# alitteneker/jsraytracer

Measured on AMD Instinct MI355X. Metric: pixel-samples/sec + %HBM-roofline, cornell_box_path 1024² @1/2/4/8 GPU, higher is better.
Workload: dtype f64; 1 GPU; cornell_box_path 1024x1024 64spp depth 8 (Incremental); width=1024, height=1024, spp=64, max_depth=8, parallelism=tiles1, col_block=1, headline=True, gather=rgba8

## Files before the change

jsraytracer_amd/csrc/device_common.h:

```cpp
#pragma once
#include <hip/hip_runtime.h>
#include <stdint.h>

#include "device_scene.h"
#include "fdlibm.h"
#include "js_number.h"

#define JSRT_HD __host__ __device__ __forceinline__

namespace jsrt {

#define JS_PI 3.141592653589793
#define DINF __builtin_inf()

JSRT_HD bool is_nan(double x) { return x != x; }
JSRT_HD double js_max(double a, double b) {
    double r = a > b ? a : b;
    if (a == b) r = __builtin_bit_cast(double, __builtin_bit_cast(uint64_t, a) & __builtin_bit_cast(uint64_t, b));
    return a != a ? a : r;
}
JSRT_HD double js_min(double a, double b) {
    double r = a < b ? a : b;
    if (a == b) r = __builtin_bit_cast(double, __builtin_bit_cast(uint64_t, a) | __builtin_bit_cast(uint64_t, b));
    return a != a ? a : r;
// ... 35 lines not shown
    if ((x == 1.0 || x == -1.0) && __builtin_isinf(y)) return __builtin_nan("");
#ifndef JSRT_LIBM_POW
    if ((x > 0.0 || (x == 0.0 && !__builtin_signbit(x))) && x <= 2.0 && y >= 1.0 && y <= 64.0 && y == floor(y))
        return pow_int_dd(x, (int)y);
#endif
    return pow(x, y);
}
__device__ __forceinline__ double js_round(double x) {
    if (!__builtin_isfinite(x) || x == 0.0) return x;
    double r = floor(x);
    if (x - r >= 0.5) r += 1.0;
    return r;
}
JSRT_HD float or0(float x) { return (x != x || x == 0.0f) ? 0.0f : x; }

__device__ __forceinline__ uint32_t mix32(uint32_t h, uint32_t v) {
    h = (h ^ v) * 0x9E3779B1u;
    h ^= h >> 15;
    h *= 0x85EBCA77u;
    h ^= h >> 13;
    return h;
}
__device__ __forceinline__ double uniform_of(uint32_t h) {
    const uint32_t hi = mix32(h, 0xA5A5A5A5u) >> 5;
    const uint32_t lo = mix32(h, 0x5A5A5A5Au) >> 6;
    return fma((double)hi, 1.0 / 134217728.0, (double)lo * (1.0 / 9007199254740992.0));
}
__device__ __forceinline__ double keyed_uniform(uint32_t pixkey, uint32_t node, uint32_t call) {
    return uniform_of(mix32(mix32(pixkey, node), call));
}
struct Rng {
    uint32_t key, node, calls;
    __device__ __forceinline__ double next() { return keyed_uniform(key, node, calls++); }
};
struct RngH {
    uint32_t h0, calls;
    __device__ __forceinline__ double next() { return uniform_of(mix32(h0, calls++)); }
};

struct F3 {
    float x, y, z;
};
JSRT_HD F3 f3(float x, float y, float z) { return F3{x, y, z}; }
JSRT_HD F3 add(F3 a, F3 b) { return f3(a.x + b.x, a.y + b.y, a.z + b.z); }
JSRT_HD F3 sub(F3 a, F3 b) { return f3(a.x - b.x, a.y - b.y, a.z - b.z); }
JSRT_HD F3 mul(F3 a, F3 b) { return f3(a.x * b.x, a.y * b.y, a.z * b.z); }
JSRT_HD F3 scale(F3 a, double s) {
    return f3((float)((double)a.x * s), (float)((double)a.y * s), (float)((double)a.z * s));
// ... 26 lines not shown
    return f3(o.x + (float)((double)d.x * t), o.y + (float)((double)d.y * t), o.z + (float)((double)d.z * t));
}
__device__ __forceinline__ void sin_cos(double x, double &s, double &c) { fdlibm::sin_cos(x, s, c); }
constexpr double SPHERE_PICK_EPS = 0x1p-44;
JSRT_HD bool f32_stable_bits(double d) {
    const uint64_t b = __builtin_bit_cast(uint64_t, d);
    const int e = (int)((uint32_t)(b >> 52) & 0x7FFu) - 1023;
    const int sh = 8 - e;
    const uint32_t m = (uint32_t)b & 0x1FFFFFFFu;
    const uint32_t dist = m > 0x10000000u ? m - 0x10000000u : 0x10000000u - m;
    return sh <= 28 && dist > (1u << (sh < 0 ? 0 : sh));
}
struct SinCos2 {
    double st, ct, sp, cp;
};
__device__ __forceinline__ void sin_cos_of_acos(double a, double &sin_phi, double &cos_phi) {
    sin_phi = sqrt((1.0 - a) * (1.0 + a));
    cos_phi = a;
}
__device__ __forceinline__ SinCos2 sphere_pick_exact(double theta, double a) {
    SinCos2 r;
    fdlibm::sin_cos(theta, r.st, r.ct);
    fdlibm::sin_cos(fdlibm::acos(a), r.sp, r.cp);
    return r;
}
template <class R>
__device__ __forceinline__ F3 sphere_pick(R &rng) {
    const double theta = 2.0 * JS_PI * rng.next();
    const double a = 2.0 * rng.next() - 1.0;
    double sin_t, cos_t, sin_phi, cos_phi;
#ifdef JSRT_EXACT_TRIG
    const bool fast = false;
#else
    sincos(theta, &sin_t, &cos_t);
    sin_cos_of_acos(a, sin_phi, cos_phi);
    const bool fast = f32_stable_bits(cos_t * sin_phi) && f32_stable_bits(cos_phi) && f32_stable_bits(sin_t * sin_phi);
#endif
    if (__builtin_expect(!fast, 0)) {
        const SinCos2 r = sphere_pick_exact(theta, a);
        sin_t = r.st, cos_t = r.ct, sin_phi = r.sp, cos_phi = r.cp;
    }
    return f3((float)(cos_t * sin_phi), or0((float)cos_phi), or0((float)(sin_t * sin_phi)));
}
template <class R>
__device__ __forceinline__ F3 sphere_pick_fast(R &rng, bool &unstable) {
    const double theta = 2.0 * JS_PI * rng.next();
    const double a = 2.0 * rng.next() - 1.0;
    double sin_t, cos_t, sin_phi, cos_phi;
    sincos(theta, &sin_t, &cos_t);
    sin_cos_of_acos(a, sin_phi, cos_phi);
    const double px = cos_t * sin_phi, pz = sin_t * sin_phi;
    unstable = !(f32_stable_bits(px) && f32_stable_bits(cos_phi) && f32_stable_bits(pz));
    return f3((float)px, or0((float)cos_phi), or0((float)pz));
}
template <class R>
__device__ __forceinline__ F3 sphere_pick_v8(R &rng) {
    const double theta = 2.0 * JS_PI * rng.next();
    const double a = 2.0 * rng.next() - 1.0;
    double sin_t, cos_t, sin_phi, cos_phi;
    fdlibm::sin_cos(theta, sin_t, cos_t);
// ... 1388 lines not shown
            const float wx = (float)((((double)n.x * Ti[0] + (double)n.y * Ti[4]) + (double)n.z * Ti[8]) + (double)nw * Ti[12]);
            const float wy = (float)((((double)n.x * Ti[1] + (double)n.y * Ti[5]) + (double)n.z * Ti[9]) + (double)nw * Ti[13]);
            const float wz = (float)((((double)n.x * Ti[2] + (double)n.y * Ti[6]) + (double)n.z * Ti[10]) + (double)nw * Ti[14]);
            wn = normalized(f3(wx, or0(wy), or0(wz)));
        } else {
            wn = f3(Lt.wn[0], Lt.wn[1], Lt.wn[2]);
            u = local.x;
            v = local.y;
        }
        L = normalized(delta);
        const double sc = (1 / (4 * JS_PI * dot3(delta, delta))) * fabs(dot3(L, wn));
        lcol = scale(mc_eval(S, Lt.color, u, v), sc);
    }
}

__device__ __forceinline__ bool path_scatter(double mirror_prob, bool has_r, F3 R, F3 N, const ShadeData &d, Rng &rng,
                                             F3 &dir, F3 &col, uint32_t &fix, bool force) {
    fix = 0;
    if (rng.next() < mirror_prob) {
        dir = R;
        col = f3(1, 1, 1);
        return has_r;
    }
    const double dp = average3(d.diff), sp = average3(d.spec);
    const double probSum = dp + sp;
    if (probSum == 0) return false;
    if (rng.next() < (dp / probSum)) {
        const uint32_t call = rng.calls;
        bool unstable;
        const F3 sp3 = sphere_pick_fast(rng, unstable);
        if (unstable || force) fix = call + 1;
        dir = normalized(add(N, sp3));
        col = scale(d.diff, 1 / JS_PI);
        return true;
    }
    dir = R;
    col = d.spec;
    return has_r;
}


__device__ __forceinline__ void camera_ray(const DCamera &C, double x, double y, Rng &rng, F3 &o, F3 &d) {
    const double *T = C.T;
    const F3 dir = f3((float)(x * C.tan_fov * C.aspect), (float)(y * C.tan_fov), -1.0f);
    o = f3((float)T[3], (float)T[7], (float)T[11]);
    d = f3((float)((((double)dir.x * T[0] + (double)dir.y * T[1]) + (double)dir.z * T[2]) + 0.0 * T[3]),
           (float)((((double)dir.x * T[4] + (double)dir.y * T[5]) + (double)dir.z * T[6]) + 0.0 * T[7]),
           (float)((((double)dir.x * T[8] + (double)dir.y * T[9]) + (double)dir.z * T[10]) + 0.0 * T[11]));
    if (C.kind == JSRT_CAMERA_DOF) {
        const double a = rng.next() * 2 * JS_PI, rr = sqrt(rng.next());
        double sa, ca;
        sin_cos(a, sa, ca);
        const float cx = (float)(rr * ca), cy = (float)(rr * sa);
// ... 25 lines not shown
```

jsraytracer_amd/csrc/device_scene.h:

```cpp
#pragma once
#include <math.h>
#include <stdint.h>

#include <cmath>

#include "../../include/jsrt_scene.h"
#include "sdf_program.h"

namespace jsrt {

enum : int32_t { INST_PRIM = 1, INST_AGG = 2, INST_BVH = 3 };

enum : int32_t { PF_BVH = 1, PF_AGG = 2, PF_SDF = 4, PF_TRI = 8 };
enum : int32_t { PF_ANALYTIC = 0, PF_MESH = PF_BVH | PF_TRI, PF_SDF_ONLY = PF_SDF, PF_ALL = 15 };
#define PF_SDF_PROFILE PF_SDF

struct DPrim {
    double inv[12];
    int32_t gkind;
    int32_t gindex;
    int32_t material;
    int32_t casts_shadow;
    float center[4];
    float half[4];
// ... 60 lines not shown
    int32_t pos_len;
    float wn[4];
    int32_t needs_uv;
    int32_t pad2[3];
    double T[16], Ti[16];
    double inv_n;
    double pad3;
};

struct DCamera {
    double T[16];
    double tan_fov, aspect, focus, sensor;
    int32_t kind, pad[3];
};

enum { MATF_UV = 1, MATF_DIFF_CONST = 2, MATF_SPEC_CONST = 4, MATF_SPEC_ZERO = 8, MATF_PUV = 16 };

struct DScene {
    const DPrim *prims;
    const DInst *insts;
    const int32_t *inst_child;
    const int32_t *roots;
    const RootBound *rbounds;
    const DRoot *rootrec;
    const double *mats;
    const double *ctx;
    const DBvhNode *bvh;
    const int32_t *leaf_prims;
    const int32_t *leaf_tris;
    const DTri *tris;
    const DTriShade *trish;
// ... 51 lines not shown
```

jsraytracer_amd/csrc/render_kernel.h:

```cpp
#pragma once
#include <hip/hip_runtime.h>
#include <stdint.h>

#include <functional>
#include <vector>

#include "device_scene.h"

namespace jsrt {

constexpr int MAX_TREE_DEPTH = 16;
constexpr int LVL_FLAG = 63;
constexpr int LVL_UNDER = 62;
static_assert(2 * MAX_TREE_DEPTH + 2 <= LVL_UNDER, "hybrid chain count pairs lvl[2L, 2L + 1] below the flags");
constexpr int BKT_N = 64;
constexpr int BKT_S = 16;
constexpr int BKT_K = BKT_N * BKT_S;
constexpr int BKT_LEVEL = 3 * BKT_K + 64;
constexpr int HAND_PLANES = 6;

struct RenderArgs {
    int32_t W, H, kind, max_depth;
    int32_t s_begin, s_end, spp;
    uint32_t seed;
// ... 31 lines not shown
    uint8_t *endl;
    uint32_t *qctr;
    uint4 *fixrec;
    uint32_t *fixctr;
    uint32_t fixcap;
    int32_t force_fix;
    float4 *sray;
    float4 *scol;
    uint32_t *bkt;
    uint32_t *bbase;
    uint32_t *brank;
    uint32_t p0, npix, s0, npaths;
    int32_t ns;
    int32_t group;
    int32_t shadow_node;
    int32_t chain;
    int32_t hybrid;
    uint32_t cap;
    int32_t bucket;
    int32_t child_sort;
    int32_t bucket_grid;
    int32_t pixel_major;
    size_t pool, level_cap;
    size_t nstride, hstride;
    size_t sstride;
};

struct RayFeed {
    const float *rays;
    const uint32_t *keys;
// ... 97 lines not shown
```

jsraytracer_amd/csrc/render_levels.h:

```cpp
#pragma once
#include <hip/hip_runtime.h>
#include <stdint.h>
#include <stdlib.h>
#include <string.h>

#include <algorithm>
#include <type_traits>
#include <vector>

#include "device_common.h"
#include "render_kernel.h"
#include "render_plan.h"

#ifndef JSRT_SHADE_OCC
#define JSRT_SHADE_OCC 4
#endif
#ifndef JSRT_SHADE_OCC_SDF
#define JSRT_SHADE_OCC_SDF 3
#endif
#ifndef JSRT_SHADE_OCC_FLAT
#define JSRT_SHADE_OCC_FLAT 5
#endif
#ifndef JSRT_SHADOW_OCC
#define JSRT_SHADOW_OCC 6
// ... 133 lines not shown

__device__ __forceinline__ void write_result(const WArgs &W, uint32_t i, F3 c) {
    const uint32_t p = W.parent[i];
    if (p == DEAD_RAY) return;
    if (p == NO_PARENT) {
        float *dst = W.root + 3 * (size_t)W.path[i];
        dst[0] = c.x;
        dst[1] = c.y;
        dst[2] = c.z;
    } else {
        W.slot[(size_t)(p & 1u) * W.nstride + (p >> 1)] = make_float4(c.x, c.y, c.z, 0.0f);
    }
}


__device__ __forceinline__ F3 pick(bool f, F3 a, F3 b) { return f3(f ? a.x : b.x, f ? a.y : b.y, f ? a.z : b.z); }
__device__ __forceinline__ Child pick(bool f, const Child &a, const Child &b) {
    return Child{pick(f, a.dir, b.dir), pick(f, a.col, b.col), pick(f, a.w, b.w), f ? a.k : b.k};
}

struct LevelRange {
    uint32_t base, count;
};
__device__ __forceinline__ LevelRange level_range(const WArgs &W, int L) {
    if (W.lvl[LVL_FLAG]) return LevelRange{0u, 0u};
    uint32_t b = 0;
    for (int j = 0; j < L; ++j) b += W.lvl[j];
    return LevelRange{b, W.lvl[L]};
}
__device__ __forceinline__ LevelRange chain_level(const WArgs &W, int L) {
    const uint32_t base = (uint32_t)L * W.cap;
    if (!W.hybrid) return LevelRange{base, W.npaths};
    if (W.lvl[LVL_FLAG]) return LevelRange{base, 0u};
    return LevelRange{base, W.lvl[2 * L] + W.lvl[2 * L + 1]};
// ... 2 lines not shown
    uint32_t c = W.npaths;
    for (int j = 1; j < L; ++j) c += as_const(W.lvl)[2 * j + 1];
    return c;
}
__device__ __forceinline__ uint32_t chain_slot(const WArgs &W, int L, uint32_t t) {
    if (!W.hybrid || L == 0) return t;
    const uint32_t nc = as_const(W.lvl)[2 * L];
    return t < nc ? ((L & 1) ? W.list1 : W.list0)[t] : side_base(W, L) + (t - nc);
}

constexpr uint32_t HAND_KR = 0x80000000u;
constexpr uint32_t HAND_DIFF = 0x40000000u;
constexpr uint32_t HAND_R = 0x20000000u;
constexpr uint32_t HAND_SPEC = 0x10000000u;
constexpr uint32_t HAND_MAT = 0x0FFFFF00u;

struct Handoff {
    F3 pos, N, R, refr, diff, spec;
    double kr;
    int32_t mkind, mat;
    uint32_t addr, key;
    uint32_t node;
    uint32_t mask;
    uint32_t flags;
};
struct NodeOut {
    F3 surf;
    uint32_t info;

    Handoff h;
// ... 155 lines not shown
        const float wx = (float)((((double)nrm.x * inv[0] + (double)nrm.y * inv[4]) + (double)nrm.z * inv[8]) + (double)nrm_w * inv[12]);
        const float wy = (float)((((double)nrm.x * inv[1] + (double)nrm.y * inv[5]) + (double)nrm.z * inv[9]) + (double)nrm_w * inv[13]);
        const float wz = (float)((((double)nrm.x * inv[2] + (double)nrm.y * inv[6]) + (double)nrm.z * inv[10]) + (double)nrm_w * inv[14]);
        sf.N = normalized(f3(wx, or0(wy), or0(wz)));
    }
    sf.u = u;
    sf.v = v;
    sf.basecolor = basecolor;
    sf.bary = bary;
    sf.has_uv = has_uv;
    sf.has_bc = has_bc;
    sf.has_bary = has_bary;
}

constexpr uint32_t INFO_FIX = 1u << 30;
template <int PF, bool TEX, bool PUV = false>
__device__ __forceinline__ int shade_node(const DScene &S, bool lit, const Hit &h, F3 o, F3 d, uint32_t addr,
                                          uint32_t key, NodeOut &out, Child &ch0, Child &ch1, uint32_t *fixl,
                                          bool force_fix) {
    const DPrim &P = S.prims[h.prim];
    Surface sf;
    const bool puv = PUV && (S.mat_flags[P.material] & MATF_PUV) != 0;
    surface_data<PF, false>(S, h, o, d, (S.mat_flags[P.material] & MATF_UV) != 0 && !puv, sf);
    const F3 N = sf.N, basecolor = sf.basecolor;
    float u = sf.u, v = sf.v;
    ShadeData sd;
    sd.pos = ray_point(o, d, h.t);
    if constexpr (PUV) {
        if (puv && (S.mat_flags[P.material] & MATF_UV)) posuv_map(S.puv[P.material], sd.pos.x, sd.pos.y, sd.pos.z, u, v);
    }
    out.h.pos = sd.pos;
// ... 60 lines not shown
    uint32_t info = INFO_HIT;
    if (lit) {
        info |= INFO_LIT;
        out.h.N = sd.N;
        out.h.R = sd.R;
        out.h.refr = sd.refr;
        out.h.diff = sd.diff;
        out.h.spec = sd.spec;
        out.h.kr = sd.kr;
        out.h.mkind = mkind;
        out.h.mat = P.material;
        const int32_t mf = S.mat_flags[P.material];
        uint32_t fl = 0;
        if (!(mf & MATF_DIFF_CONST) || sf.has_bc) fl |= HAND_DIFF;
        if (!(mf & MATF_SPEC_CONST)) fl |= HAND_SPEC;
        if (mkind != JSRT_MAT_PHONG && sd.kr != 1.0) fl |= HAND_KR | HAND_R;
        if (!(mf & MATF_SPEC_ZERO) || !(__builtin_isfinite(sd.R.x) && __builtin_isfinite(sd.R.y) && __builtin_isfinite(sd.R.z)))
            fl |= HAND_R;
        out.h.flags = fl;
        rng.calls = (uint32_t)S.light_draws;
    }
    int n = 0;
    uint32_t fix0 = 0u, fix1 = 0u;
    auto push = [&](const Child &c) {
        const bool first = n == 0;
        ch0 = pick(first, c, ch0);
        ch1 = pick(first, ch1, c);
        ++n;
    };
    if (mkind == JSRT_MAT_PHONG) {
        if (dot3(sd.refl, sd.refl) > 0) push(Child{sd.R, f3(1, 1, 1), sd.refl, 1.0});
        if (dot3(sd.trans, sd.trans) > 0) push(Child{normalized(d), f3(1, 1, 1), sd.trans, 1.0});
    } else {
        if (sd.kr > 0) {
            F3 dir = sd.R, col = f3(1, 1, 1);
            bool ok = true;
            uint32_t fx = 0;
            if (mkind == JSRT_MAT_PATH) ok = path_scatter(M.mirror_prob, true, sd.R, Nn, sd, rng, dir, col, fx, force_fix);
            if (ok) {
                fix0 = fx;
                push(Child{dir, col, sd.refl, sd.kr});
            }
        }
        if (sd.kr < 1) {
            F3 dir = sd.refr, col = f3(1, 1, 1);
            bool ok = sd.has_refr;
            uint32_t fx = 0;
            if (mkind == JSRT_MAT_PATH) ok = path_scatter(M.mirror_prob, sd.has_refr, sd.refr, neg(Nn), sd, rng, dir, col, fx, force_fix);
            if (ok) {
                if (fx) {
                    if (n == 0) fix0 = fx | 0x80000000u;
                    else fix1 = fx | 0x80000000u;
                }
                push(Child{dir, col, sd.trans, 1 - sd.kr});
            }
        }
    }
    if (__builtin_expect((fix0 | fix1) != 0u, 0)) {
        const uint32_t t = threadIdx.x;
        fixl[t] = fix0;
        fixl[256 + t] = fix1;
        fixl[512 + t] = __float_as_uint(Nn.x);
        fixl[768 + t] = __float_as_uint(Nn.y);
        fixl[1024 + t] = __float_as_uint(Nn.z);
        info |= INFO_FIX;
    }
    out.info = info | ((uint32_t)n << INFO_NCHILD_SHIFT);
    return n;
}

__device__ __forceinline__ float u2f(uint32_t x) { return __uint_as_float(x); }
__device__ __forceinline__ uint32_t f2u(float x) { return __float_as_uint(x); }

// ... 6 lines not shown
__device__ __forceinline__ void store_child(const WArgs &W, uint32_t i, uint32_t j, const Child &c) {
    float4 *x = W.child + (size_t)(2 * j) * W.nstride + i;
    x[0] = make_float4(c.col.x, c.col.y, c.col.z, c.w.x);
    if (!unit_child(c))
        x[W.nstride] = make_float4(c.w.y, c.w.z, u2f((uint32_t)__double2loint(c.k)), u2f((uint32_t)__double2hiint(c.k)));
}
__device__ __forceinline__ F3 add_child(const WArgs &W, uint32_t i, uint32_t j, F3 c, F3 v, uint32_t info,
                                       const float4 *first = nullptr) {
    const float4 *x = W.child + (size_t)(2 * j) * W.nstride + i;
    const float4 a = first ? *first : x[0];
    if (info & (j == 0 ? INFO_UNIT0 : INFO_UNIT1)) return add(c, mul(v, f3(a.x, a.y, a.z)));
    const float4 b = x[W.nstride];
    const double k = __hiloint2double((int)f2u(b.w), (int)f2u(b.z));
    return add(c, scale(mul(mul(v, f3(a.x, a.y, a.z)), f3(a.w, b.x, b.y)), k));
}
__device__ __forceinline__ void store_hand(const WArgs &W, uint32_t h, const Handoff &o) {
    float4 *p = W.hand + h;
    const size_t hs = W.hstride;
    const uint32_t fl = o.flags;
    const uint32_t tag = ((uint32_t)o.mat << 8) | (o.mask & 0xFFu) | fl;
    p[0] = make_float4(o.pos.x, o.pos.y, o.pos.z, u2f(mix32(o.key, o.addr)));
    p[hs] = make_float4(o.N.x, o.N.y, o.N.z, u2f(tag));
    if (fl & HAND_DIFF) p[2 * hs] = make_float4(o.diff.x, o.diff.y, o.diff.z, 0.0f);
    if (fl & HAND_R) p[3 * hs] = make_float4(o.R.x, o.R.y, o.R.z, u2f((uint32_t)__double2hiint(o.kr)));
    if (fl & HAND_SPEC) p[4 * hs] = make_float4(o.spec.x, o.spec.y, o.spec.z, 0.0f);
    if (fl & HAND_KR) p[5 * hs] = make_float4(o.refr.x, o.refr.y, o.refr.z, u2f((uint32_t)__double2loint(o.kr)));
    if (W.bucket) W.hnode[h] = o.node;
}

__device__ __forceinline__ F3 accumulate(const RenderArgs &A, F3 acc, F3 col) {
    if (A.kind == JSRT_RENDERER_RANDOM) return add(acc, scale(col, 1.0 / A.spp));
    if (A.kind == JSRT_RENDERER_INCREMENTAL) return f3(acc.x + col.x, acc.y + or0(col.y), acc.z + or0(col.z));
    return col;
}

// ... 120 lines not shown
    SL.prims = reinterpret_cast<const DPrim *>(sb + SL.stab_off[STAB_PRIMS]);
    SL.prim_shade = reinterpret_cast<const int32_t *>(sb + SL.stab_off[STAB_PRIM_SHADE]);
    SL.shade0 = reinterpret_cast<const double *>(sb + SL.stab_off[STAB_SHADE0]);
    SL.shadeI = reinterpret_cast<const double *>(sb + SL.stab_off[STAB_SHADEI]);
    SL.prim_lit = reinterpret_cast<const int32_t *>(sb + SL.stab_off[STAB_PRIM_LIT]);
    SL.puv = reinterpret_cast<const jsrt_rec_posuv *>(sb + SL.stab_off[STAB_POSUV]);
}
__device__ __forceinline__ void stab_stage(const DScene &S, DScene &SL, int words, bool shade) {
    extern __shared__ uint4 stab_lds[];
    const uint4 *src = reinterpret_cast<const uint4 *>(S.stab);
    for (int k = (int)threadIdx.x; k < words; k += 256) stab_lds[k] = src[k];
    __syncthreads();
    stab_bind(SL, stab_lds, shade);
}

template <int PF, bool CHAIN, bool STAGE, bool TEX = false, bool PUV = false>
__global__ __launch_bounds__(256, PF == PF_ANALYTIC ? JSRT_SHADE_OCC_FLAT
                                                    : (PF & PF_SDF) ? JSRT_SHADE_OCC_SDF : JSRT_SHADE_OCC) SHADE_ATTR void k_shade(
    DScene S, WArgs W, int L, int child_depth) {
    const uint32_t t0 = blockIdx.x * 256, tt = t0 + threadIdx.x;
    const LevelRange R = CHAIN ? chain_level(W, L) : level_range(W, L);
    const uint32_t count = R.count, base = R.base, next_base = CHAIN ? 0u : R.base + R.count;
    if (!CHAIN || W.hybrid || STAGE) {
        if (t0 >= count) return;
    } else if (tt >= count) {
        return;
    }
    const bool in = tt < count;
    const uint32_t q = in ? tt : 0u;
    const uint32_t slot = CHAIN && in ? chain_slot(W, L, q) : q;
    const uint32_t i = base + (CHAIN ? slot : q);
    const uint32_t r = CHAIN ? slot : i;
    int nchild = 0;
    Child ch0, ch1;
// ... 18 lines not shown
    uint32_t parent = 0, path = 0, hslot = ~0u;
    if (!CHAIN && prim != NO_RAY) {
        parent = W.parent[r];
        path = W.path[r];
    }
    if (hit) {
        if (!STAGE) {
            ro = f3(W.ox[r], W.oy[r], W.oz[r]);
            rd = f3(W.dx[r], W.dy[r], W.dz[r]);
            rt = W.t[r];
            rctx = W.ctx[r];
            raddr = W.addr[r];
            rkey = W.key[r];
        }
        const Hit h{rt, prim, rctx};
        nchild = shade_node<PF, TEX, PUV>(SL, W.ns > 0, h, ro, rd, raddr, rkey, out, ch0, ch1, fixl, W.force_fix != 0);
        out.h.node = CHAIN ? slot : q;
        out.h.mask = (uint32_t)S.grid_cells;
        if (W.bucket && (out.info & INFO_LIT)) {
            const uint32_t br = W.brank[r];
            const int b = (int)(br >> 16);
            const uint32_t *B = W.bkt + (size_t)L * BKT_LEVEL;
            hslot = B[2 * BKT_K + bucket_key(W, b)] + W.bbase[(size_t)blockIdx.x * BKT_N + b] + (br & 0xFFFFu);
            if (hslot >= B[3 * BKT_K]) hslot = ~0u;
            if (W.bucket_grid) out.h.mask = (uint32_t)b;
        }
    }
    uint32_t co[2] = {0u, 1u};
    uint32_t at = 0, side_at = 0;
    if (!CHAIN) {
        const int nc = child_depth > 0 ? nchild : 0;
        if (W.child_sort)
            at = block_append_keyed(W.lvl + L + 1, nc, nchild > 0 ? octant(ch0.dir) : 0, nchild > 1 ? octant(ch1.dir) : 0,
                                    co[0], co[1]);
        else
            at = block_append<256>(W.lvl + L + 1, nc);
    } else if (W.hybrid) {
        const int side = (child_depth > 0 && nchild > 1) ? 1 : 0, cont = (child_depth > 0 && nchild > 0) ? 1 : 0;
        block_append2(W.lvl + 2 * (L + 1), cont, side, at, side_at);
        side_at += side_base(W, L + 1);
    }
    if (__builtin_expect(hit && (out.info & INFO_FIX) != 0u, 0) && child_depth > 0) {
        if (CHAIN) fix_record(W, fixl, out.h.key, out.h.addr, W.hybrid ? nchild : 1, r, side_at);
        else fix_record(W, fixl, out.h.key, out.h.addr, nchild, next_base + at + co[0], next_base + at + co[1]);
    }
    if (prim == NO_RAY) {
        if (in) store_node(W, i, f3(0, 0, 0), 0u);
        if (CHAIN && W.hybrid && in) W.endl[r] = (uint8_t)L;
        return;
    }
    if (!hit) {
        const F3 bg = f3(S.bg[0], S.bg[1], S.bg[2]);
        if (CHAIN) {
            store_node(W, i, bg, INFO_MISS);
            W.prim[r] = NO_RAY;
            if (W.hybrid) W.endl[r] = (uint8_t)L;
        } else {
            if (parent == NO_PARENT) {
                float *dst = W.root + 3 * (size_t)path;
                dst[0] = bg.x;
                dst[1] = bg.y;
                dst[2] = bg.z;
            } else if (parent != DEAD_RAY) {
                W.slot[(size_t)(parent & 1u) * W.nstride + (parent >> 1)] = make_float4(bg.x, bg.y, bg.z, 0.0f);
            }
            store_node(W, i, bg, 0u);
        }
        return;
    }
    if (nchild > 0 && unit_child(ch0)) out.info |= INFO_UNIT0;
    if (nchild > 1 && unit_child(ch1)) out.info |= INFO_UNIT1;
    store_node(W, i, out.surf, out.info & ~INFO_FIX);
    if (out.info & INFO_LIT) {
        if (!W.bucket) store_hand(W, q, out.h);
        else if (hslot != ~0u) store_hand(W, hslot, out.h);
    }
    if (nchild > 0) store_child(W, i, 0, ch0);
    if (nchild > 1) store_child(W, i, 1, ch1);
    if (CHAIN) {
        uint32_t *next = (L & 1) ? W.list0 : W.list1;
        if (child_depth > 0 && nchild > 0) {
            W.ox[r] = out.h.pos.x; W.oy[r] = out.h.pos.y; W.oz[r] = out.h.pos.z;
            W.dx[r] = ch0.dir.x; W.dy[r] = ch0.dir.y; W.dz[r] = ch0.dir.z;
            W.addr[r] = mix32(out.h.addr, 1u);
            if (W.hybrid) next[at] = r;
        } else {
            W.prim[r] = NO_RAY;
            if (W.hybrid) W.endl[r] = (uint8_t)L;
        }
        if (W.hybrid && child_depth > 0 && nchild > 1) {
// ... 29 lines not shown
        W.dx[rr] = c.dir.x; W.dy[rr] = c.dir.y; W.dz[rr] = c.dir.z;
        W.addr[rr] = mix32(out.h.addr, (uint32_t)j + 1);
        W.key[rr] = out.h.key;
        W.path[rr] = path;
        W.parent[rr] = 2 * i + (uint32_t)j;
        W.prim[rr] = -1;
    }
}


__device__ __forceinline__ F3 mc_const3(const DScene &S, int m) {
    const float4 c = *reinterpret_cast<const float4 *>(S.mc_const + 4 * m);
    return f3(c.x, c.y, c.z);
}
__device__ __forceinline__ bool hand_decode(const DScene &S, const float4 &h1, const float4 *hp, size_t hs, ShadeData &sd,
                                            int &mkind) {
    const uint32_t tag = f2u(h1.w);
    const jsrt_rec_material &M = S.mat[(tag & HAND_MAT) >> 8];
    sd.N = f3(h1.x, h1.y, h1.z);
    sd.diff = (tag & HAND_DIFF) ? f3(hp[2 * hs].x, hp[2 * hs].y, hp[2 * hs].z) : mc_const3(S, M.diffuse);
    sd.spec = (tag & HAND_SPEC) ? f3(hp[4 * hs].x, hp[4 * hs].y, hp[4 * hs].z) : mc_const3(S, M.specular);
    sd.R = f3(0, 0, 0);
    sd.refr = f3(0, 0, 0);
    sd.kr = 1.0;
    if (tag & HAND_R) {
        const float4 h3 = hp[3 * hs];
        sd.R = f3(h3.x, h3.y, h3.z);
        if (tag & HAND_KR) {
            const float4 h5 = hp[5 * hs];
            sd.refr = f3(h5.x, h5.y, h5.z);
            sd.kr = __hiloint2double((int)f2u(h3.w), (int)f2u(h5.w));
        }
    }
// ... 124 lines not shown
    const LevelRange R = CHAIN ? chain_level(W, L) : level_range(W, L);
    const uint32_t count = R.count, base = R.base;
    const uint32_t ns = (uint32_t)W.ns;
    const uint32_t e = blockIdx.x * 256 + threadIdx.x;
    const bool in = e < as_const(W.bkt + (size_t)L * BKT_LEVEL)[3 * BKT_K];
    const uint32_t h = in ? e : 0u;
    const float4 *hp = W.hand + h;
    const size_t hs = W.hstride;
    const uint32_t q = W.hnode[h];
    const float4 h0 = hp[0], h1 = hp[hs];
    const uint32_t tag = f2u(h1.w);
    uint64_t mask = ~0ull;
    if (W.bucket_grid && S.grid_masked) mask = wave_root_mask(S, tag & 0xFFu, in);
    const bool lit = in && q < (CHAIN ? W.cap : count);
    const uint32_t i = base + (lit ? q : 0u);
    const float4 nd = W.node[i];
    DScene SL = S;
    stab_stage(S, SL, S.stab_words_shadow, false);
    if (!lit) return;
    const F3 P = f3(h0.x, h0.y, h0.z);
    ShadeData sd;
    int mkind;
    const bool no_r = hand_decode(SL, h1, hp, hs, sd, mkind);
    F3 d[NS], c[NS];
    uint32_t live = 0u;
#pragma unroll
    for (int s = 0; s < NS; ++s) {
        d[s] = f3(1, 1, 1);
        c[s] = f3(0, 0, 0);
        if ((uint32_t)s < ns) {
            RngH rng{f2u(h0.w), (uint32_t)SL.sample_call[s]};
            F3 Ld, lcol;
            light_sample<false>(SL, as_const(S.lights)[0], P, rng, d[s], Ld, lcol);
            c[s] = light_sample_color(mkind, sd, Ld, lcol, no_r);
            if (!(c[s].x == 0.0f && c[s].y == 0.0f && c[s].z == 0.0f)) live |= 1u << s;
        }
    }
    live = world_any_node<PF, NS>(S, P, d, live, 0.0001, 1, mask);
// ... 270 lines not shown
            v = sf.v;
            hu = 1;
        }
    }
    uv[2 * (size_t)i] = u;
    uv[2 * (size_t)i + 1] = v;
    has[i] = hu;
}
template <int PF>
void material_uv_pf(const DScene &S, const float *rays, uint32_t n, float *uv, int32_t *has, hipStream_t st) {
    const size_t lds = (PF & (PF_BVH | PF_AGG)) ? bvh_lds_bytes(S, 256) : 0;
    hipLaunchKernelGGL((k_material_uv<PF>), dim3(grid_ub(n)), dim3(256), lds, st, S, rays, n, uv, has);
}

template <int PF, bool CHAIN>
void run_batch(const DScene &S, const RenderArgs &A, const WArgs &W, hipStream_t st, KernelTimes *kt,
               const std::vector<size_t> &bound, const BatchSync *sync) {
    auto accum_wait = [&] { if (sync && sync->wait) (void)hipStreamWaitEvent(st, sync->wait, 0); };
    auto accum_done = [&] { if (sync && sync->done) (void)hipEventRecord(sync->done, st); };
    const hipStream_t ss = (sync && sync->aux) ? sync->aux : st;
    const bool split = ss != st;
    auto timed = [&](int which, auto launch) {
        const bool ev = kt && kt->on(which);
        const hipStream_t s = which == KT_SHADOW ? ss : st;
        if (ev) kt->ev[which].begin(s);
        launch();
        if (ev) kt->ev[which].end(s);
    };
    const size_t lds = (PF & (PF_BVH | PF_AGG)) ? bvh_lds_bytes(S, 256) : 0;
    const bool Q = (PF & PF_SDF) && W.sstride != 0;
    if (Q) (void)hipMemsetAsync(W.qctr, 0, 64 * sizeof(uint32_t), st);
    if (W.bucket) (void)hipMemsetAsync(W.bkt, 0, (size_t)MAX_TREE_DEPTH * BKT_LEVEL * sizeof(uint32_t), st);
// ... 13 lines not shown
        timed(KT_EXTEND, [&] {
            if (Q && S.sdf_all_forms)
                hipLaunchKernelGGL((k_extend_q<PF, CHAIN, true>), dim3(persistent_grid((const void *)k_extend_q<PF, CHAIN, true>, ub)),
                                   dim3(256), 0, st, S, W, L, L == 0 ? 0.0 : 0.0001);
            else if (Q)
                hipLaunchKernelGGL((k_extend_q<PF, CHAIN, false>), dim3(persistent_grid((const void *)k_extend_q<PF, CHAIN, false>, ub)),
                                   dim3(256), 0, st, S, W, L, L == 0 ? 0.0 : 0.0001);
            else
                hipLaunchKernelGGL((k_extend<PF, CHAIN>), dim3(grid_ub(ub)), dim3(256), lds, st, S, W, L, L == 0 ? 0.0 : 0.0001);
        });
        if (W.bucket) hipLaunchKernelGGL(k_bucket_offsets, dim3(1), dim3(256), 0, st, W, L);
        if (split && L > 0 && W.ns > 0) (void)hipStreamWaitEvent(st, sync->shadow_done, 0);
        timed(KT_SHADE, [&] {
            const bool staged = PF == PF_ANALYTIC && S.stab_words > 0;
            const size_t sl = staged ? (size_t)S.stab_words * 16 : 0;
            if (S.has_posuv) {
                if (staged)
                    hipLaunchKernelGGL((k_shade<PF, CHAIN, PF == PF_ANALYTIC, true, true>), dim3(grid_ub(ub)), dim3(256), sl, st, S, W, L, child_depth);
                else
                    hipLaunchKernelGGL((k_shade<PF, CHAIN, false, true, true>), dim3(grid_ub(ub)), dim3(256), 0, st, S, W, L, child_depth);
            } else if (S.has_textures) {
                if (staged)
                    hipLaunchKernelGGL((k_shade<PF, CHAIN, PF == PF_ANALYTIC, true>), dim3(grid_ub(ub)), dim3(256), sl, st, S, W, L, child_depth);
                else
                    hipLaunchKernelGGL((k_shade<PF, CHAIN, false, true>), dim3(grid_ub(ub)), dim3(256), 0, st, S, W, L, child_depth);
            } else if (staged)
                hipLaunchKernelGGL((k_shade<PF, CHAIN, PF == PF_ANALYTIC>), dim3(grid_ub(ub)), dim3(256), sl, st, S, W, L, child_depth);
            else
                hipLaunchKernelGGL((k_shade<PF, CHAIN, false>), dim3(grid_ub(ub)), dim3(256), 0, st, S, W, L, child_depth);
            if (child_depth > 0) hipLaunchKernelGGL(k_fix_dirs, dim3(1), dim3(256), 0, st, W);
// ... 19 lines not shown
                const size_t sl = (size_t)S.stab_words_shadow * 16;
                auto shadow = [&](auto serial, auto stage) {
                    constexpr bool SERIAL = decltype(serial)::value, STAGE = decltype(stage)::value;
                    const dim3 g(grid_ub(SERIAL ? ub : ne));
                    const size_t l = STAGE ? sl : lds;
                    if (S.sphere_lights)
                        hipLaunchKernelGGL((k_shadow<PF, CHAIN, SERIAL, true, STAGE>), g, dim3(256), l, ss, S, W, L);
                    else
                        hipLaunchKernelGGL((k_shadow<PF, CHAIN, SERIAL, false, STAGE>), g, dim3(256), l, ss, S, W, L);
                };
                constexpr bool FLAT_PF = PF == PF_ANALYTIC;
                if (W.ns > 1 && W.group <= 1) {
                    shadow(std::true_type{}, std::false_type{});
                } else if (FLAT_PF && sl) {
                    if constexpr (FLAT_PF) {
                        if (W.shadow_node && W.bucket && S.n_lights == 1 && !S.sphere_lights && W.ns > 1 && W.ns <= 4) {
                            hipLaunchKernelGGL((k_shadow_node<PF, CHAIN, 4>), dim3(grid_ub(ub)), dim3(256), sl, ss, S, W, L);
                            return;
                        }
                    }
                    shadow(std::false_type{}, std::bool_constant<FLAT_PF>{});
                } else {
                    shadow(std::false_type{}, std::false_type{});
                }
            });
        if (W.ns > 0 && split) (void)hipEventRecord(sync->shadow_done, ss);
    }
    if (split && W.ns > 0 && !ubs.empty()) (void)hipStreamWaitEvent(st, sync->shadow_done, 0);
    if (CHAIN && W.hybrid) {
        timed(KT_RESOLVE, [&] {
            if (ubs.empty()) {
// ... 36 lines not shown
```

jsraytracer_amd/csrc/scene_load.cpp:

```cpp
#include "scene_load.h"

#include <float.h>
#include <math.h>
#include <string.h>

#include <algorithm>
#include <map>
#include <set>
#include <unordered_map>

namespace jsrt {
namespace {

struct Blob {
    const jsrt_rec_renderer *rndr = nullptr;
    const jsrt_rec_camera *cam = nullptr;
    const jsrt_rec_mcolor *mc = nullptr;
    const jsrt_rec_material *mat = nullptr;
    const jsrt_rec_geometry *geom = nullptr;
    const jsrt_rec_object *obj = nullptr;
    const jsrt_rec_matrix *mats = nullptr;
    const int32_t *root = nullptr, *chld = nullptr;
    const jsrt_rec_bvhnode *bvh = nullptr;
    const jsrt_rec_triangle *tri = nullptr;
// ... 1029 lines not shown
                check_mc((int32_t)i);
                S.has_textures = 1;
            }
        }
        if (S.has_textures) {
            S.tex.assign(B.tex, B.tex + B.n_tex);
            S.texels.assign(B.texl, B.texl + B.n_texl);
            for (int b = 0; b < 256; ++b) S.tex_q255.push_back((double)b / 255.0);
        }
        mc_constants();
        for (size_t i = 0; i < S.mat.size(); ++i) {
            const jsrt_rec_material &M = S.mat[i];
            if (M.kind == JSRT_MAT_SOLID || M.kind == JSRT_MAT_TRANSPARENT) continue;
            const float *d = &S.mc_const[4 * (size_t)M.diffuse], *sp = &S.mc_const[4 * (size_t)M.specular];
            if (d[3] != 0.0f) S.mat_flags[i] |= MATF_DIFF_CONST;
            if (sp[3] != 0.0f) {
                S.mat_flags[i] |= MATF_SPEC_CONST;
                uint32_t b[3];
                memcpy(b, sp, sizeof b);
                if (b[0] == 0u && b[1] == 0u && b[2] == 0u && M.smoothness >= 0.0 && M.smoothness <= 1e5)
                    S.mat_flags[i] |= MATF_SPEC_ZERO;
            }
        }

        const double I[16] = {1, 0, 0, 0, 0, 1, 0, 0, 0, 0, 1, 0, 0, 0, 0, 1};
        for (int k = 0; k < 16; ++k) S.ctx.push_back(I[k]);
        S.all_roots_prims = 1;
        for (uint32_t i = 0; i < B.n_root; ++i) {
            const int32_t ix = inst(B.root[i], I, 0);
            S.roots.push_back(ix);
// ... 248 lines not shown
```

Before: 676.7 million pixel-samples/s.

## Skip node store via handoff tag packing and specialize last-level shade kernel

For the analytic flat pipeline with a single light and bucketed shadow-node path, the shade kernel now packs the child count and unit bits, plus an ambient-needed flag, into the handoff tag. The shadow-node kernel rebuilds the node word from that tag and from the constant material ambient, so the separate node store and load is skipped when ambient is constant. A LAST template specialization of k_shade for child_depth==0 skips child appends, fix records and direction sampling while still advancing the RNG call counter. The price is more template instantiations and a tighter material-index field in the tag.

```diff
diff --git a/jsraytracer_amd/csrc/device_common.h b/jsraytracer_amd/csrc/device_common.h
--- a/jsraytracer_amd/csrc/device_common.h
+++ b/jsraytracer_amd/csrc/device_common.h
@@ -73,24 +73,24 @@
 }
 JSRT_HD float or0(float x) { return (x != x || x == 0.0f) ? 0.0f : x; }
 
-__device__ __forceinline__ uint32_t mix32(uint32_t h, uint32_t v) {
+JSRT_HD uint32_t mix32(uint32_t h, uint32_t v) {
     h = (h ^ v) * 0x9E3779B1u;
     h ^= h >> 15;
     h *= 0x85EBCA77u;
     h ^= h >> 13;
     return h;
 }
-__device__ __forceinline__ double uniform_of(uint32_t h) {
+JSRT_HD double uniform_of(uint32_t h) {
     const uint32_t hi = mix32(h, 0xA5A5A5A5u) >> 5;
     const uint32_t lo = mix32(h, 0x5A5A5A5Au) >> 6;
     return fma((double)hi, 1.0 / 134217728.0, (double)lo * (1.0 / 9007199254740992.0));
 }
-__device__ __forceinline__ double keyed_uniform(uint32_t pixkey, uint32_t node, uint32_t call) {
+JSRT_HD double keyed_uniform(uint32_t pixkey, uint32_t node, uint32_t call) {
     return uniform_of(mix32(mix32(pixkey, node), call));
 }
 struct Rng {
     uint32_t key, node, calls;
-    __device__ __forceinline__ double next() { return keyed_uniform(key, node, calls++); }
+    JSRT_HD double next() { return keyed_uniform(key, node, calls++); }
 };
 struct RngH {
     uint32_t h0, calls;
@@ -147,7 +147,7 @@
 struct SinCos2 {
     double st, ct, sp, cp;
 };
-__device__ __forceinline__ void sin_cos_of_acos(double a, double &sin_phi, double &cos_phi) {
+JSRT_HD void sin_cos_of_acos(double a, double &sin_phi, double &cos_phi) {
     sin_phi = sqrt((1.0 - a) * (1.0 + a));
     cos_phi = a;
 }
@@ -176,7 +176,7 @@
     return f3((float)(cos_t * sin_phi), or0((float)cos_phi), or0((float)(sin_t * sin_phi)));
 }
 template <class R>
-__device__ __forceinline__ F3 sphere_pick_fast(R &rng, bool &unstable) {
+JSRT_HD F3 sphere_pick_fast(R &rng, bool &unstable) {
     const double theta = 2.0 * JS_PI * rng.next();
     const double a = 2.0 * rng.next() - 1.0;
     double sin_t, cos_t, sin_phi, cos_phi;
@@ -1595,8 +1595,9 @@
     }
 }
 
-__device__ __forceinline__ bool path_scatter(double mirror_prob, bool has_r, F3 R, F3 N, const ShadeData &d, Rng &rng,
-                                             F3 &dir, F3 &col, uint32_t &fix, bool force) {
+template <bool NODIR = false>
+JSRT_HD bool path_scatter(double mirror_prob, bool has_r, F3 R, F3 N, const ShadeData &d, Rng &rng, F3 &dir, F3 &col,
+                          uint32_t &fix, bool force) {
     fix = 0;
     if (rng.next() < mirror_prob) {
         dir = R;
@@ -1607,17 +1608,71 @@
     const double probSum = dp + sp;
     if (probSum == 0) return false;
     if (rng.next() < (dp / probSum)) {
-        const uint32_t call = rng.calls;
-        bool unstable;
-        const F3 sp3 = sphere_pick_fast(rng, unstable);
-        if (unstable || force) fix = call + 1;
-        dir = normalized(add(N, sp3));
+        if constexpr (NODIR) {
+            rng.calls += 2;
+            dir = N;
+        } else {
+            const uint32_t call = rng.calls;
+            bool unstable;
+            const F3 sp3 = sphere_pick_fast(rng, unstable);
+            if (unstable || force) fix = call + 1;
+            dir = normalized(add(N, sp3));
+        }
         col = scale(d.diff, 1 / JS_PI);
         return true;
     }
     dir = R;
     col = d.spec;
     return has_r;
+}
+
+JSRT_HD F3 pick(bool f, F3 a, F3 b) { return f3(f ? a.x : b.x, f ? a.y : b.y, f ? a.z : b.z); }
+JSRT_HD Child pick(bool f, const Child &a, const Child &b) {
+    return Child{pick(f, a.dir, b.dir), pick(f, a.col, b.col), pick(f, a.w, b.w), f ? a.k : b.k};
+}
+template <bool NODIR = false>
+JSRT_HD int scatter_children(int mkind, double mirror_prob, const ShadeData &sd, F3 d, Rng &rng, bool force_fix,
+                             Child &ch0, Child &ch1, uint32_t &fix0, uint32_t &fix1) {
+    const F3 Nn = sd.N;
+    int n = 0;
+    fix0 = 0u;
+    fix1 = 0u;
+    auto push = [&](const Child &c) {
+        const bool first = n == 0;
+        ch0 = pick(first, c, ch0);
+        ch1 = pick(first, ch1, c);
+        ++n;
+    };
+    if (mkind == JSRT_MAT_PHONG) {
+        if (dot3(sd.refl, sd.refl) > 0) push(Child{sd.R, f3(1, 1, 1), sd.refl, 1.0});
+        if (dot3(sd.trans, sd.trans) > 0) push(Child{NODIR ? sd.R : normalized(d), f3(1, 1, 1), sd.trans, 1.0});
+    } else {
+        if (sd.kr > 0) {
+            F3 dir = sd.R, col = f3(1, 1, 1);
+            bool ok = true;
+            uint32_t fx = 0;
+            if (mkind == JSRT_MAT_PATH) ok = path_scatter<NODIR>(mirror_prob, true, sd.R, Nn, sd, rng, dir, col, fx, force_fix);
+            if (ok) {
+                fix0 = fx;
+                push(Child{dir, col, sd.refl, sd.kr});
+            }
+        }
+        if (sd.kr < 1) {
+            F3 dir = sd.refr, col = f3(1, 1, 1);
+            bool ok = sd.has_refr;
+            uint32_t fx = 0;
+            if (mkind == JSRT_MAT_PATH)
+                ok = path_scatter<NODIR>(mirror_prob, sd.has_refr, sd.refr, neg(Nn), sd, rng, dir, col, fx, force_fix);
+            if (ok) {
+                if (fx) {
+                    if (n == 0) fix0 = fx | 0x80000000u;
+                    else fix1 = fx | 0x80000000u;
+                }
+                push(Child{dir, col, sd.trans, 1 - sd.kr});
+            }
+        }
+    }
+    return n;
 }
 
 
diff --git a/jsraytracer_amd/csrc/device_scene.h b/jsraytracer_amd/csrc/device_scene.h
--- a/jsraytracer_amd/csrc/device_scene.h
+++ b/jsraytracer_amd/csrc/device_scene.h
@@ -98,7 +98,7 @@
     int32_t kind, pad[3];
 };
 
-enum { MATF_UV = 1, MATF_DIFF_CONST = 2, MATF_SPEC_CONST = 4, MATF_SPEC_ZERO = 8, MATF_PUV = 16 };
+enum { MATF_UV = 1, MATF_DIFF_CONST = 2, MATF_SPEC_CONST = 4, MATF_SPEC_ZERO = 8, MATF_PUV = 16, MATF_AMB_CONST = 32 };
 
 struct DScene {
     const DPrim *prims;
diff --git a/jsraytracer_amd/csrc/render_kernel.h b/jsraytracer_amd/csrc/render_kernel.h
--- a/jsraytracer_amd/csrc/render_kernel.h
+++ b/jsraytracer_amd/csrc/render_kernel.h
@@ -69,6 +69,7 @@
     int32_t ns;
     int32_t group;
     int32_t shadow_node;
+    int32_t node_single;
     int32_t chain;
     int32_t hybrid;
     uint32_t cap;
diff --git a/jsraytracer_amd/csrc/render_levels.h b/jsraytracer_amd/csrc/render_levels.h
--- a/jsraytracer_amd/csrc/render_levels.h
+++ b/jsraytracer_amd/csrc/render_levels.h
@@ -171,10 +171,6 @@
 }
 
 
-__device__ __forceinline__ F3 pick(bool f, F3 a, F3 b) { return f3(f ? a.x : b.x, f ? a.y : b.y, f ? a.z : b.z); }
-__device__ __forceinline__ Child pick(bool f, const Child &a, const Child &b) {
-    return Child{pick(f, a.dir, b.dir), pick(f, a.col, b.col), pick(f, a.w, b.w), f ? a.k : b.k};
-}
 
 struct LevelRange {
     uint32_t base, count;
@@ -207,6 +203,18 @@
 constexpr uint32_t HAND_R = 0x20000000u;
 constexpr uint32_t HAND_SPEC = 0x10000000u;
 constexpr uint32_t HAND_MAT = 0x0FFFFF00u;
+constexpr uint32_t HAND_MAT1 = 0x007FFF00u;
+constexpr uint32_t HAND_AMB = 0x00800000u;
+constexpr int HAND_INFO_SHIFT = 24;
+static_assert((size_t)STAB_MAX_WORDS * 16 / sizeof(int32_t) <= (HAND_MAT1 >> 8) + 1, "a staged scene's materials fit HAND_MAT1");
+static_assert(INFO_NCHILD_SHIFT == 2 && INFO_UNIT0 == 32u && INFO_UNIT1 == 64u, "hand_info's packing");
+__device__ __forceinline__ uint32_t hand_info(uint32_t info) {
+    return (((info >> INFO_NCHILD_SHIFT) & 3u) | ((info >> 3) & 0xCu)) << HAND_INFO_SHIFT;
+}
+__device__ __forceinline__ uint32_t hand_info_word(uint32_t tag) {
+    const uint32_t p = tag >> HAND_INFO_SHIFT;
+    return INFO_HIT | INFO_LIT | ((p & 3u) << INFO_NCHILD_SHIFT) | ((p & 0xCu) << 3);
+}
 
 struct Handoff {
     F3 pos, N, R, refr, diff, spec;
@@ -392,7 +400,7 @@
 }
 
 constexpr uint32_t INFO_FIX = 1u << 30;
-template <int PF, bool TEX, bool PUV = false>
+template <int PF, bool TEX, bool PUV = false, bool NODIR = false>
 __device__ __forceinline__ int shade_node(const DScene &S, bool lit, const Hit &h, F3 o, F3 d, uint32_t addr,
                                           uint32_t key, NodeOut &out, Child &ch0, Child &ch1, uint32_t *fixl,
                                           bool force_fix) {
@@ -483,49 +491,55 @@
         uint32_t fl = 0;
         if (!(mf & MATF_DIFF_CONST) || sf.has_bc) fl |= HAND_DIFF;
         if (!(mf & MATF_SPEC_CONST)) fl |= HAND_SPEC;
+        if constexpr (PF == PF_ANALYTIC)
+            if (!(mf & MATF_AMB_CONST) || sf.has_bc) fl |= HAND_AMB;
         if (mkind != JSRT_MAT_PHONG && sd.kr != 1.0) fl |= HAND_KR | HAND_R;
         if (!(mf & MATF_SPEC_ZERO) || !(__builtin_isfinite(sd.R.x) && __builtin_isfinite(sd.R.y) && __builtin_isfinite(sd.R.z)))
             fl |= HAND_R;
         out.h.flags = fl;
         rng.calls = (uint32_t)S.light_draws;
     }
+    uint32_t fix0 = 0u, fix1 = 0u;
     int n = 0;
-    uint32_t fix0 = 0u, fix1 = 0u;
-    auto push = [&](const Child &c) {
-        const bool first = n == 0;
-        ch0 = pick(first, c, ch0);
-        ch1 = pick(first, ch1, c);
-        ++n;
-    };
-    if (mkind == JSRT_MAT_PHONG) {
-        if (dot3(sd.refl, sd.refl) > 0) push(Child{sd.R, f3(1, 1, 1), sd.refl, 1.0});
-        if (dot3(sd.trans, sd.trans) > 0) push(Child{normalized(d), f3(1, 1, 1), sd.trans, 1.0});
+    if constexpr (PF == PF_ANALYTIC) {
+        n = scatter_children<NODIR>(mkind, M.mirror_prob, sd, d, rng, force_fix, ch0, ch1, fix0, fix1);
     } else {
-        if (sd.kr > 0) {
-            F3 dir = sd.R, col = f3(1, 1, 1);
-            bool ok = true;
-            uint32_t fx = 0;
-            if (mkind == JSRT_MAT_PATH) ok = path_scatter(M.mirror_prob, true, sd.R, Nn, sd, rng, dir, col, fx, force_fix);
-            if (ok) {
-                fix0 = fx;
-                push(Child{dir, col, sd.refl, sd.kr});
+        auto push = [&](const Child &c) {
+            const bool first = n == 0;
+            ch0 = pick(first, c, ch0);
+            ch1 = pick(first, ch1, c);
+            ++n;
+        };
+        if (mkind == JSRT_MAT_PHONG) {
+            if (dot3(sd.refl, sd.refl) > 0) push(Child{sd.R, f3(1, 1, 1), sd.refl, 1.0});
+            if (dot3(sd.trans, sd.trans) > 0) push(Child{normalized(d), f3(1, 1, 1), sd.trans, 1.0});
+        } else {
+            if (sd.kr > 0) {
+                F3 dir = sd.R, col = f3(1, 1, 1);
+                bool ok = true;
+                uint32_t fx = 0;
+                if (mkind == JSRT_MAT_PATH) ok = path_scatter(M.mirror_prob, true, sd.R, Nn, sd, rng, dir, col, fx, force_fix);
+                if (ok) {
+                    fix0 = fx;
+                    push(Child{dir, col, sd.refl, sd.kr});
+                }
             }
-        }
-        if (sd.kr < 1) {
-            F3 dir = sd.refr, col = f3(1, 1, 1);
-            bool ok = sd.has_refr;
-            uint32_t fx = 0;
-            if (mkind == JSRT_MAT_PATH) ok = path_scatter(M.mirror_prob, sd.has_refr, sd.refr, neg(Nn), sd, rng, dir, col, fx, force_fix);
-            if (ok) {
-                if (fx) {
-                    if (n == 0) fix0 = fx | 0x80000000u;
-                    else fix1 = fx | 0x80000000u;
+            if (sd.kr < 1) {
+                F3 dir = sd.refr, col = f3(1, 1, 1);
+                bool ok = sd.has_refr;
+                uint32_t fx = 0;
+                if (mkind == JSRT_MAT_PATH) ok = path_scatter(M.mirror_prob, sd.has_refr, sd.refr, neg(Nn), sd, rng, dir, col, fx, force_fix);
+                if (ok) {
+                    if (fx) {
+                        if (n == 0) fix0 = fx | 0x80000000u;
+                        else fix1 = fx | 0x80000000u;
+                    }
+                    push(Child{dir, col, sd.trans, 1 - sd.kr});
                 }
-                push(Child{dir, col, sd.trans, 1 - sd.kr});
             }
         }
     }
-    if (__builtin_expect((fix0 | fix1) != 0u, 0)) {
+    if (!NODIR && __builtin_expect((fix0 | fix1) != 0u, 0)) {
         const uint32_t t = threadIdx.x;
         fixl[t] = fix0;
         fixl[256 + t] = fix1;
@@ -562,11 +576,13 @@
     const double k = __hiloint2double((int)f2u(b.w), (int)f2u(b.z));
     return add(c, scale(mul(mul(v, f3(a.x, a.y, a.z)), f3(a.w, b.x, b.y)), k));
 }
-__device__ __forceinline__ void store_hand(const WArgs &W, uint32_t h, const Handoff &o) {
+template <bool FLAT>
+__device__ __forceinline__ void store_hand(const WArgs &W, uint32_t h, const Handoff &o, uint32_t info) {
     float4 *p = W.hand + h;
     const size_t hs = W.hstride;
-    const uint32_t fl = o.flags;
-    const uint32_t tag = ((uint32_t)o.mat << 8) | (o.mask & 0xFFu) | fl;
+    const uint32_t fl = FLAT ? o.flags & ~HAND_AMB : o.flags;
+    uint32_t tag = ((uint32_t)o.mat << 8) | (o.mask & 0xFFu) | fl;
+    if (FLAT && W.node_single) tag |= (o.flags & HAND_AMB) | hand_info(info);
     p[0] = make_float4(o.pos.x, o.pos.y, o.pos.z, u2f(mix32(o.key, o.addr)));
     p[hs] = make_float4(o.N.x, o.N.y, o.N.z, u2f(tag));
     if (fl & HAND_DIFF) p[2 * hs] = make_float4(o.diff.x, o.diff.y, o.diff.z, 0.0f);
@@ -717,10 +733,11 @@
     stab_bind(SL, stab_lds, shade);
 }
 
-template <int PF, bool CHAIN, bool STAGE, bool TEX = false, bool PUV = false>
+template <int PF, bool CHAIN, bool STAGE, bool TEX = false, bool PUV = false, bool LAST = false>
 __global__ __launch_bounds__(256, PF == PF_ANALYTIC ? JSRT_SHADE_OCC_FLAT
                                                     : (PF & PF_SDF) ? JSRT_SHADE_OCC_SDF : JSRT_SHADE_OCC) SHADE_ATTR void k_shade(
-    DScene S, WArgs W, int L, int child_depth) {
+    DScene S, WArgs W, int L, int child_depth_arg) {
+    const int child_depth = LAST ? 0 : child_depth_arg;
     const uint32_t t0 = blockIdx.x * 256, tt = t0 + threadIdx.x;
     const LevelRange R = CHAIN ? chain_level(W, L) : level_range(W, L);
     const uint32_t count = R.count, base = R.base, next_base = CHAIN ? 0u : R.base + R.count;
@@ -769,7 +786,7 @@
             rkey = W.key[r];
         }
         const Hit h{rt, prim, rctx};
-        nchild = shade_node<PF, TEX, PUV>(SL, W.ns > 0, h, ro, rd, raddr, rkey, out, ch0, ch1, fixl, W.force_fix != 0);
+        nchild = shade_node<PF, TEX, PUV, LAST>(SL, W.ns > 0, h, ro, rd, raddr, rkey, out, ch0, ch1, fixl, W.force_fix != 0);
         out.h.node = CHAIN ? slot : q;
         out.h.mask = (uint32_t)S.grid_cells;
         if (W.bucket && (out.info & INFO_LIT)) {
@@ -783,7 +800,8 @@
     }
     uint32_t co[2] = {0u, 1u};
     uint32_t at = 0, side_at = 0;
-    if (!CHAIN) {
+    if (LAST) {
+    } else if (!CHAIN) {
         const int nc = child_depth > 0 ? nchild : 0;
         if (W.child_sort)
             at = block_append_keyed(W.lvl + L + 1, nc, nchild > 0 ? octant(ch0.dir) : 0, nchild > 1 ? octant(ch1.dir) : 0,
@@ -795,7 +813,7 @@
         block_append2(W.lvl + 2 * (L + 1), cont, side, at, side_at);
         side_at += side_base(W, L + 1);
     }
-    if (__builtin_expect(hit && (out.info & INFO_FIX) != 0u, 0) && child_depth > 0) {
+    if (!LAST && __builtin_expect(hit && (out.info & INFO_FIX) != 0u, 0) && child_depth > 0) {
         if (CHAIN) fix_record(W, fixl, out.h.key, out.h.addr, W.hybrid ? nchild : 1, r, side_at);
         else fix_record(W, fixl, out.h.key, out.h.addr, nchild, next_base + at + co[0], next_base + at + co[1]);
     }
@@ -825,10 +843,12 @@
     }
     if (nchild > 0 && unit_child(ch0)) out.info |= INFO_UNIT0;
     if (nchild > 1 && unit_child(ch1)) out.info |= INFO_UNIT1;
-    store_node(W, i, out.surf, out.info & ~INFO_FIX);
-    if (out.info & INFO_LIT) {
-        if (!W.bucket) store_hand(W, q, out.h);
-        else if (hslot != ~0u) store_hand(W, hslot, out.h);
+    const uint32_t info = out.info & ~INFO_FIX;
+    const bool by_shadow = PF == PF_ANALYTIC && W.node_single && (info & INFO_LIT) && !(out.h.flags & HAND_AMB) && hslot != ~0u;
+    if (!by_shadow) store_node(W, i, out.surf, info);
+    if (info & INFO_LIT) {
+        if (!W.bucket) store_hand<PF == PF_ANALYTIC>(W, q, out.h, info);
+        else if (hslot != ~0u) store_hand<PF == PF_ANALYTIC>(W, hslot, out.h, info);
     }
     if (nchild > 0) store_child(W, i, 0, ch0);
     if (nchild > 1) store_child(W, i, 1, ch1);
@@ -888,9 +908,9 @@
     return f3(c.x, c.y, c.z);
 }
 __device__ __forceinline__ bool hand_decode(const DScene &S, const float4 &h1, const float4 *hp, size_t hs, ShadeData &sd,
-                                            int &mkind) {
+                                            int &mkind, uint32_t matmask = HAND_MAT) {
     const uint32_t tag = f2u(h1.w);
-    const jsrt_rec_material &M = S.mat[(tag & HAND_MAT) >> 8];
+    const jsrt_rec_material &M = S.mat[(tag & matmask) >> 8];
     sd.N = f3(h1.x, h1.y, h1.z);
     sd.diff = (tag & HAND_DIFF) ? f3(hp[2 * hs].x, hp[2 * hs].y, hp[2 * hs].z) : mc_const3(S, M.diffuse);
     sd.spec = (tag & HAND_SPEC) ? f3(hp[4 * hs].x, hp[4 * hs].y, hp[4 * hs].z) : mc_const3(S, M.specular);
@@ -1045,14 +1065,23 @@
     if (W.bucket_grid && S.grid_masked) mask = wave_root_mask(S, tag & 0xFFu, in);
     const bool lit = in && q < (CHAIN ? W.cap : count);
     const uint32_t i = base + (lit ? q : 0u);
-    const float4 nd = W.node[i];
+    const bool single = W.node_single != 0;
+    float4 nd = make_float4(0.0f, 0.0f, 0.0f, 0.0f);
+    if (!single || (lit && (tag & HAND_AMB))) nd = W.node[i];
     DScene SL = S;
     stab_stage(S, SL, S.stab_words_shadow, false);
     if (!lit) return;
     const F3 P = f3(h0.x, h0.y, h0.z);
     ShadeData sd;
     int mkind;
-    const bool no_r = hand_decode(SL, h1, hp, hs, sd, mkind);
+    const bool no_r = hand_decode(SL, h1, hp, hs, sd, mkind, single ? HAND_MAT1 : HAND_MAT);
+    if (single) {
+        if (!(tag & HAND_AMB)) {
+            const F3 amb = mc_const3(SL, SL.mat[(tag & HAND_MAT1) >> 8].ambient);
+            nd.x = amb.x, nd.y = amb.y, nd.z = amb.z;
+        }
+        nd.w = u2f(hand_info_word(tag));
+    }
     F3 d[NS], c[NS];
     uint32_t live = 0u;
 #pragma unroll
@@ -1353,8 +1382,12 @@
 }
 
 template <int PF, bool CHAIN>
-void run_batch(const DScene &S, const RenderArgs &A, const WArgs &W, hipStream_t st, KernelTimes *kt,
+void run_batch(const DScene &S, const RenderArgs &A, const WArgs &pool_args, hipStream_t st, KernelTimes *kt,
                const std::vector<size_t> &bound, const BatchSync *sync) {
+    const bool node_form = PF == PF_ANALYTIC && S.stab_words_shadow > 0 && pool_args.shadow_node && pool_args.bucket &&
+                           S.n_lights == 1 && !S.sphere_lights && pool_args.ns > 1 && pool_args.ns <= 4 && pool_args.group > 1;
+    WArgs W = pool_args;
+    W.node_single = node_form ? 1 : 0;
     auto accum_wait = [&] { if (sync && sync->wait) (void)hipStreamWaitEvent(st, sync->wait, 0); };
     auto accum_done = [&] { if (sync && sync->done) (void)hipEventRecord(sync->done, st); };
     const hipStream_t ss = (sync && sync->aux) ? sync->aux : st;
@@ -1398,6 +1431,20 @@
         timed(KT_SHADE, [&] {
             const bool staged = PF == PF_ANALYTIC && S.stab_words > 0;
             const size_t sl = staged ? (size_t)S.stab_words * 16 : 0;
+            if constexpr (PF == PF_ANALYTIC) {
+                if (child_depth == 0) {
+                    auto last = [&](auto stage, auto tex, auto puv) {
+                        constexpr bool ST = decltype(stage)::value, TX = decltype(tex)::value, PU = decltype(puv)::value;
+                        hipLaunchKernelGGL((k_shade<PF, CHAIN, ST, TX, PU, true>), dim3(grid_ub(ub)), dim3(256), ST ? sl : 0, st, S, W, L, 0);
+                    };
+                    using T = std::true_type;
+                    using F = std::false_type;
+                    if (S.has_posuv) staged ? last(T{}, T{}, T{}) : last(F{}, T{}, T{});
+                    else if (S.has_textures) staged ? last(T{}, T{}, F{}) : last(F{}, T{}, F{});
+                    else staged ? last(T{}, F{}, F{}) : last(F{}, F{}, F{});
+                    return;
+                }
+            }
             if (S.has_posuv) {
                 if (staged)
                     hipLaunchKernelGGL((k_shade<PF, CHAIN, PF == PF_ANALYTIC, true, true>), dim3(grid_ub(ub)), dim3(256), sl, st, S, W, L, child_depth);
@@ -1447,7 +1494,7 @@
                     shadow(std::true_type{}, std::false_type{});
                 } else if (FLAT_PF && sl) {
                     if constexpr (FLAT_PF) {
-                        if (W.shadow_node && W.bucket && S.n_lights == 1 && !S.sphere_lights && W.ns > 1 && W.ns <= 4) {
+                        if (node_form) {
                             hipLaunchKernelGGL((k_shadow_node<PF, CHAIN, 4>), dim3(grid_ub(ub)), dim3(256), sl, ss, S, W, L);
                             return;
                         }
diff --git a/jsraytracer_amd/csrc/scene_load.cpp b/jsraytracer_amd/csrc/scene_load.cpp
--- a/jsraytracer_amd/csrc/scene_load.cpp
+++ b/jsraytracer_amd/csrc/scene_load.cpp
@@ -1067,6 +1067,7 @@
             if (M.kind == JSRT_MAT_SOLID || M.kind == JSRT_MAT_TRANSPARENT) continue;
             const float *d = &S.mc_const[4 * (size_t)M.diffuse], *sp = &S.mc_const[4 * (size_t)M.specular];
             if (d[3] != 0.0f) S.mat_flags[i] |= MATF_DIFF_CONST;
+            if (S.mc_const[4 * (size_t)M.ambient + 3] != 0.0f) S.mat_flags[i] |= MATF_AMB_CONST;
             if (sp[3] != 0.0f) {
                 S.mat_flags[i] |= MATF_SPEC_CONST;
                 uint32_t b[3];
```

Measured after the change: 684.3 million pixel-samples/s (median of 6 runs). 1.1% higher.
